# tmaklin/ntcomp

Hardware: AMD Instinct MI355X
Metric: encode Mbases/sec at k=91, 150bp reads, 1/2/4/8 MI355X; bit-exact vs CPU (higher is better)
Workload: dtype u32; 1 GPU; C91: 10000000 x 150bp synthetic reads per GPU (1% subst, 50% revcomp) vs SBWT of a 5 Mbp synthetic genome (+revcomp), k=91; k=91, read_len=150, genome_bp=5000000, err_ppm=10000, reads_per_gpu=10000000, batch_reads=10000000, index_nodes=10000001, records_per_gpu=39278538, suffix_table_u=14, spill_reruns=0, parallelism=reads sharded over 1 GPU(s), index replicated, no collective, inflight=2

## Files before the change

### ntcomp_amd/csrc/capi.cpp

```cpp
#include <hip/hip_runtime.h>

#include <algorithm>
#include <chrono>
#include <cstdio>
#include <cstdlib>
#include <cstring>
#include <exception>
#include <memory>
#include <string>
#include <vector>

#include "../../include/ntcomp_gpu.h"
#include "../../include/ntcomp_codec.h"
#include "../../include/ntcomp_host.h"
#include "codec_params.h"
#include "derived.h"
#include "kernels.h"
#include "nonacgt_core.h"
#include "qrans_core.h"
#include "quality_core.h"
#include "names_core.h"
#include "digest_core.h"
#include "pair_core.h"
#include "window_core.h"
// ... 132 lines not shown
    Enc4Args last4{};
    struct {
        const uint8_t *bases;
        const uint64_t *offs;
        uint64_t n_reads, total_bases, cap;
        uint64_t *rec_out, *rec_offs;
    } call4{};
    uint32_t ent_slots_opt = 0;
    double epool_per_read = 4.0;
    double rpool_per_read = 1.0;
    double epool_per_base = 0.0;
    double rpool_per_base = 0.0;
    uint64_t spill_reruns = 0;
    uint32_t tab_u_opt = 0;
    int tab_u_fallback = 0;
    int pair_bytes_opt = 1;
    int filter_opt = -1;
    int64_t filter_density_ppm = -1;
    int joint_opt = -1;
    int path_link_opt = path_link_on() ? 1 : 0;
    int win_opt = -1;
    int subst_opt = subst_on() ? -1 : 0;
    int subst_built = 0;
    int decode_only_opt = 0;
    bool index_decode_only = false;
    int ext2_opt = 0;
    uint64_t n_paths = 0, path_text_len = 0;
    int64_t upload_host_us = 0, upload_total_us = 0;
    uint64_t max_pass_bases = 1ULL << 30;
    double last_pack_ms = 0;
    NxState nx;
    QualState qual;
    NameState names;
    DigestState dig;
    PairState pair;
    WindowState win;
    int discard_text = 0;
    FastqArgs fq_last{};
    hipEvent_t pack_ev[3] = {nullptr, nullptr, nullptr};
};

namespace {

constexpr uint64_t kCounterBytes = 8 * 64 + 2 * 64;

#define HIP_TRY(ctx, expr)                                                                   \
// ... 1092 lines not shown

int ntc_index_upload(ntc_ctx *ctx, const ntc_index_view *v) {
    if (!ctx || !view_ok(v)) return set_err(ctx, NTC_ERR_INVALID_ARG, "null index view");
    ntc_index_prep p;
    std::string err;
    const int rc = prepare_index(v, p, err);
    if (rc) return set_err(ctx, rc, err);
    return upload_prepared(ctx, p);
}

}

namespace {
struct Upload {
    ntc_ctx *ctx;
    const HostIndex &hx;
    const Derived &dv;
    const uint64_t n;
    const int64_t host_us;
    const std::chrono::steady_clock::time_point t_start = std::chrono::steady_clock::now();
    void *d_lines = nullptr, *d_lcs = nullptr, *d_uniq = nullptr, *d_walk = nullptr;
    void *d_walk_a = nullptr, *d_walk_b = nullptr, *d_pred = nullptr, *d_code = nullptr;
    void *d_pstream = nullptr, *d_colex_at = nullptr, *d_pos = nullptr, *d_puniq = nullptr;
    bool has_paths = false;
    uint64_t tlen = 0, n_paths = 0;
    uint32_t U = 0;
    void *d_tab = nullptr, *d_bits = nullptr, *d_fbits = nullptr;

    Upload(ntc_ctx *c, const ntc_index_prep &p) : ctx(c), hx(p.hx), dv(p.dv), n(p.hx.n), host_us(p.host_us) {}
    int dalloc(uint64_t bytes, void **p) {
        HIP_TRY(ctx, hipMalloc(p, bytes));
        ctx->index_mem->ptrs.push_back(*p);
        ctx->index_bytes += bytes;
        return NTC_OK;
    }
    double seconds() const { return std::chrono::duration<double>(std::chrono::steady_clock::now() - t_start).count(); }
    void mark(const char *what, bool sync) const {
        static const bool trace = std::getenv("NTC_UPLOAD_TRACE") != nullptr;
        if (!trace) return;
        if (sync) (void)hipStreamSynchronize(ctx->stream);
        std::fprintf(stderr, "[upload] %-28s %.4f s\n", what, seconds());
    }
};

int up_free_previous(Upload &u) {
    ntc_ctx *ctx = u.ctx;
    HIP_TRY(ctx, hipStreamSynchronize(ctx->stream));
// ... 98 lines not shown
        uint32_t np32 = 0;
        HIP_TRY(ctx, hipMemcpyAsync(&u.tlen, (uint64_t *)d_base + n, 8, hipMemcpyDeviceToHost, ctx->stream));
        HIP_TRY(ctx, hipMemcpyAsync(&np32, cnt + 1, 4, hipMemcpyDeviceToHost, ctx->stream));
        HIP_TRY(ctx, hipStreamSynchronize(ctx->stream));
        HIP_TRY(ctx, hipGetLastError());
        u.n_paths = np32;
        const uint64_t tlen = u.tlen;
        if (tlen + 64 < (1ULL << 31)) {
            const uint64_t n_groups = (tlen + hx.k) / 32 + 8, n_colex = tlen + 8, n_puniq = tlen / 64 + 4;
            if ((rc = u.dalloc(n_puniq * 8, &u.d_puniq)) || (rc = u.dalloc(n_groups * 16, &u.d_pstream)) ||
                (rc = u.dalloc(n_colex * 4 + 64, &u.d_colex_at)) || (rc = u.dalloc(n * 4, &u.d_pos))) {
                free_tmp();
                return rc;
            }
            HIP_TRY(ctx, hipMemsetAsync(u.d_puniq, 0, n_puniq * 8, ctx->stream));
            HIP_TRY(ctx, hipMemsetAsync(u.d_pstream, 0, n_groups * 16, ctx->stream));
            HIP_TRY(ctx, hipMemsetAsync(u.d_colex_at, 0xFF, n_colex * 4 + 64, ctx->stream));
            HIP_TRY(ctx, hipMemsetAsync(u.d_pos, 0xFF, n * 4, ctx->stream));
            launch_path_place(pa, st, prv, (const uint64_t *)d_base, (uint32_t *)u.d_colex_at, (uint32_t *)u.d_pos,
                              (uint4 *)u.d_pstream, (uint64_t *)u.d_puniq, ctx->stream);
            if (hx.k >= kForkBlockMinK)
                launch_path_forks(pa, st, (const uint32_t *)d_len, (const uint64_t *)d_base, (const uint32_t *)u.d_pos,
                                  (const uint4 *)u.d_pstream, (uint32_t *)u.d_colex_at, ctx->stream);
            HIP_TRY(ctx, hipGetLastError());
            u.has_paths = true;
        }
        free_tmp();
    }
    u.mark("path cover", true);
    HIP_TRY(ctx, hipStreamSynchronize(ctx->stream));
    HIP_TRY(ctx, hipFree(u.d_walk_a));
    HIP_TRY(ctx, hipFree(u.d_walk_b));
    HIP_TRY(ctx, hipFree(u.d_pred));
    HIP_TRY(ctx, hipFree(u.d_code));
    return NTC_OK;
}

int up_joint_choice(Upload &u) {
    ntc_ctx *ctx = u.ctx;
    const bool has_paths = u.has_paths;
    DevIndex &d = ctx->dix;
    d = DevIndex{};
    d.rank = (const uint2 *)u.d_lines;
    d.lcs = (const uint8_t *)u.d_lcs;
    d.uniq = (const uint32_t *)u.d_uniq;
    d.walk = (const WalkEntry *)u.d_walk;
    d.rwords = u.dv.rwords;
    d.n = (uint32_t)u.n;
    d.k = u.hx.k;
    d.t_jump = u.dv.t_jump;
    for (int c = 0; c < 5; c++) d.C[c] = u.dv.C[c];
    d.has_paths = has_paths ? 1u : 0u;
    d.path_len = has_paths ? (uint32_t)u.tlen : 0u;
    d.pstream = (const uint4 *)u.d_pstream;
    d.colex_at = (const uint32_t *)u.d_colex_at;
    d.pos_of_node = (const uint32_t *)u.d_pos;
    d.puniq = (const uint64_t *)u.d_puniq;
    d.forks = has_paths && u.hx.k >= kForkBlockMinK ? 1u : 0u;
    d.absent = u.dv.absent;
    d.joint = has_paths && (ctx->joint_opt == 1 || (ctx->joint_opt < 0 && u.n_paths * kJointAutoNodesPerPath > u.n))
                  ? 1u : 0u;
    return NTC_OK;
}

int up_suffix_table(Upload &u) {
    ntc_ctx *ctx = u.ctx;
    DevIndex &d = ctx->dix;
    const uint64_t n = u.n;
    int rc;
    if (ctx->ext2_opt) {
        void *d_r2;
        if ((rc = u.dalloc(rank2_blocks(n) * 4 * sizeof(Rank2Chunk), &d_r2))) return rc;
        launch_rank2(d, (Rank2Chunk *)d_r2, ctx->stream);
        d.rank2 = (const Rank2Chunk *)d_r2;
    }
    uint32_t U = ctx->tab_u_opt ? std::min<uint32_t>(ctx->tab_u_opt, std::min<uint32_t>(u.hx.k, kTabMaxU))
                                : default_tab_u(n, u.hx.k, u.hx.lcs.data());
    ctx->tab_u_fallback = 0;
    if (!ctx->tab_u_opt && U > 14) {
        size_t free_b = 0, total_b = 0;
        if (hipMemGetInfo(&free_b, &total_b) == hipSuccess &&
// ... 172 lines not shown
    uint64_t t = 0;
    for (const auto &b : ctx->ws) t += b.bytes;
    *value = (int64_t)t;
    return NTC_OK;
}

#define OPT_SET(member) [](ntc_ctx *c, int64_t v) { c->member = (decltype(c->member))v; return (int)NTC_OK; }
#define OPT_GET(expr) [](const ntc_ctx *c, int64_t *v) { *v = (int64_t)(expr); return (int)NTC_OK; }
#define OPT_VALUE(member) OPT_SET(member), OPT_GET(c->member)
#define OPT_UPLOAD(member, built) OPT_SET(member), OPT_GET(c->has_index ? (int64_t)(built) : (int64_t)c->member)
#define OPT_READ(key, expr) {key, 0, 0, kInRange, nullptr, nullptr, OPT_GET(expr)}
#define OPT_DEV(f) {"dev_" #f, 0, 0, kInRange, nullptr, nullptr, \
                    [](const ntc_ctx *c, int64_t *v) { return get_dev_addr(c, c->dix.f, v); }}

const Option kOptions[] = {
    {"encode_variant", 1, 4, kEndsOnly, "encode_variant must be 4 (default) or 1 (A/B baseline)", OPT_VALUE(encode_variant)},
    {"tab_u", 0, kTabMaxU, kInRange, "tab_u must be 0 (default) or 1..15", OPT_UPLOAD(tab_u_opt, c->dix.tab_u)},
    {"pair_bytes", 0, 1, kInRange, "pair_bytes must be 0 or 1", OPT_UPLOAD(pair_bytes_opt, c->dix.pair_w != nullptr)},
    {"filter", -1, 1, kInRange, "filter must be -1 (auto), 0 or 1", OPT_UPLOAD(filter_opt, c->dix.filt_f != 0)},
    {"joint", -1, 1, kInRange, "joint must be -1 (auto), 0 or 1", OPT_UPLOAD(joint_opt, c->dix.joint)},
    {"path_link", 0, 1, kInRange, "path_link must be 0 or 1", OPT_VALUE(path_link_opt)},
    {"win", -1, 1, kInRange, "win must be -1 (auto), 0 or 1", OPT_UPLOAD(win_opt, c->dix.win_w != nullptr)},
    {"subst", -1, 0, kInRange, "subst must be -1 (auto) or 0", OPT_UPLOAD(subst_opt, c->subst_built)},
    {"decode_only", 0, 1, kInRange, "decode_only must be 0 or 1", OPT_UPLOAD(decode_only_opt, c->index_decode_only)},
    {"ext2", 0, 1, kInRange, "ext2 must be 0 or 1", OPT_UPLOAD(ext2_opt, c->dix.rank2 != nullptr)},
    {"warm_dma", 1, 1ll << 30, kInRange, "warm_dma: 1 .. 2^30 bytes", warm_dma, nullptr},
    {"max_pass_bases", 1, kNoMax, kInRange, "max_pass_bases must be >= 1", OPT_VALUE(max_pass_bases)},
    {"ent_slots", 0, 1024, kMultipleOf4, "ent_slots must be 0 (auto) or a multiple of 4 up to 1024", OPT_SET(ent_slots_opt),
     OPT_GET(ent_slots(c))},
    {"pool_per_read", 0, kNoMax, kInRange, "pool_per_read must be >= 0", set_pool_per_read, nullptr},
    {"qualities", 0, 2, kInRange, "qualities must be 0 (drop), 1 (keep) or 2 (bin8)", OPT_VALUE(qual.mode)},
    {"quality_coder", 0, 1, kInRange, "quality_coder must be 0 (pack) or 1 (rans)", OPT_VALUE(qual.coder)},
    {"names", 0, 2, kInRange, "names must be 0 (drop), 1 (keep) or 2 (id)", OPT_VALUE(names.mode)},
    {"discard_text", 0, 1, kInRange, "discard_text must be 0 or 1", OPT_VALUE(discard_text)},
    {"paired", 0, 2, kInRange, "paired must be 0 (off), 1 (ids) or 2 (no check)", OPT_VALUE(pair.mode)},
    {"digests", 0, 1, kInRange, "digests must be 0 or 1", OPT_VALUE(dig.opt)},
    {"non_acgt", 0, 2, kInRange, "non_acgt must be 0 (error), 1 (mask) or 2 (keep)", OPT_VALUE(nx.policy)},
    {"subst_hash", 0, 0, kInRange, nullptr, nullptr, get_subst_hash},
    {"path_hash", 0, 0, kInRange, nullptr, nullptr, get_path_hash},
    {"workspace_bytes", 0, 0, kInRange, nullptr, nullptr, get_workspace_bytes},
    OPT_DEV(walk), OPT_DEV(rank2), OPT_DEV(tab), OPT_DEV(tab_bits),
    OPT_DEV(filt_bits),
    OPT_DEV(pair_w), OPT_DEV(win_w),
    OPT_READ("filter_density_ppm", c->filter_density_ppm),
    OPT_READ("n_paths", c->n_paths),
    OPT_READ("path_text_len", c->path_text_len),
// ... 1517 lines not shown
```

### ntcomp_amd/csrc/derived.cpp

```cpp
#include "derived.h"

#include <algorithm>
#include <cmath>
#include <cstdlib>
#include <string>
#include <thread>

namespace ntc {

bool build_derived(const HostIndex &ix, Derived &out, std::string &err, bool host_paths) {
    const uint64_t n = ix.n;
    const uint32_t k = ix.k;
    if (n == 0 || n >= (uint64_t)kTabShort) {
        err = "index must have 1 <= n < 2^32 - 256 nodes";
        return false;
    }
    if (k < 1 || k > 255) {
        err = "k must be in [1, 255]";
        return false;
    }
    const uint64_t nw = (n + 63) / 64;
    for (int c = 0; c < 4; c++)
        if (ix.rows[c].size() < nw) {
            err = "subset-matrix row shorter than ceil(n/64) words";
// ... 174 lines not shown
    if (!head || !alone || m == 0 || (m & (m - 1))) return kNoNode;
    const int c = __builtin_ctz(m);
    const uint32_t y = dv.C[c] + host_rank(dv, c, z);
    return dummy[y] ? kNoNode : y;
}

void fork_words(const HostIndex &ix, const Derived &dv, const std::vector<uint8_t> &dummy, uint32_t v, uint32_t *w) {
    uint64_t h = v;
    while (h > 0 && ix.lcs[h] >= ix.k - 1) h--;
    const uint32_t m = labels_of(dv, h);
    for (int c = 0; c < 4; c++) {
        w[c] = kNoNode;
        if (!((m >> c) & 1u)) continue;
        const uint32_t y = dv.C[c] + host_rank(dv, c, h);
        if (!dummy[y]) w[c] = dv.pos_of_node[y];
    }
}

bool subst_on() {
    const char *e = std::getenv("NTC_SUBST");
    return !(e && std::atoi(e) == 0);
}

bool path_link_on() {
    const char *e = std::getenv("NTC_PATH_LINK");
    return !(e && std::atoi(e) == 0);
}

void link_unitigs(const HostIndex &ix, const Derived &dv, const std::vector<uint8_t> &dummy,
                  std::vector<uint32_t> &nxt, std::vector<uint32_t> &prv) {
    const uint64_t n = ix.n;
    const uint32_t k = ix.k;
    std::vector<uint32_t> ulen(n, 0);
    for (uint64_t z = 1; z < n; z++) {
        if (dummy[z] || prv[z] != kNoNode) continue;
        uint32_t c = 0;
        for (uint32_t y = (uint32_t)z; y != kNoNode; y = nxt[y]) c++;
        for (uint32_t y = (uint32_t)z; y != kNoNode; y = nxt[y]) ulen[y] = c;
    }
    std::vector<uint64_t> best_pred(n, UINT64_MAX);
    std::vector<uint32_t> want(n, kNoNode);
    for (uint64_t t = 1; t < n; t++) {
        if (dummy[t] || !ulen[t] || nxt[t] != kNoNode) continue;
        uint64_t h = t;
        while (h > 0 && ix.lcs[h] >= k - 1) h--;
        const uint32_t m = labels_of(dv, h);
        uint64_t best = UINT64_MAX;
        const uint64_t mine = (uint64_t)ulen[t] << 32 | t;
        for (int c = 0; c < 4; c++) {
            if (!((m >> c) & 1u)) continue;
            const uint32_t y = dv.C[c] + host_rank(dv, c, h);
            if (dummy[y] || prv[y] != kNoNode || !ulen[y]) continue;
            best = std::min(best, (uint64_t)ulen[y] << 32 | y);
            best_pred[y] = std::min(best_pred[y], mine);
        }
        if (best != UINT64_MAX) want[t] = (uint32_t)best;
    }
    for (uint64_t t = 1; t < n; t++) {
        const uint32_t y = want[t];
        if (y != kNoNode && best_pred[y] == ((uint64_t)ulen[t] << 32 | t)) {
            nxt[t] = y;
            prv[y] = (uint32_t)t;
        }
    }
}

void build_paths(const HostIndex &ix, Derived &dv) {
    const uint64_t n = ix.n;
    const uint32_t k = ix.k;
    dv.has_paths = false;
    if (n >= (1ULL << 31) || k < 1) return;
    const std::vector<uint8_t> dummy = dummy_nodes(ix, dv);
    std::vector<uint32_t> nxt(n), prv(n, kNoNode);
    for (uint64_t z = 0; z < n; z++) {
        nxt[z] = path_succ(ix, dv, dummy, z);
        if (nxt[z] != kNoNode) prv[nxt[z]] = (uint32_t)z;
    }
    if (path_link_on()) link_unitigs(ix, dv, dummy, nxt, prv);
    std::vector<uint8_t> start(n, 0), seen(n, 0);
    for (uint64_t z = 1; z < n; z++)
        if (!dummy[z] && prv[z] == kNoNode) {
            start[z] = 1;
            for (uint32_t y = (uint32_t)z; y != kNoNode; y = nxt[y]) seen[y] = 1;
        }
    for (uint64_t z = 1; z < n; z++)
        if (!dummy[z] && !seen[z]) {
            start[z] = 1;
            for (uint32_t y = (uint32_t)z; !seen[y]; y = nxt[y]) seen[y] = 1;
        }
    std::vector<uint64_t> path_start;
    std::vector<uint32_t> order;
    order.reserve(n);
    for (uint64_t z = 1; z < n; z++) {
// ... 20 lines not shown
    uint64_t b = 0;
    std::vector<uint8_t> first(k);
    for (uint64_t p = 0; p < np; p++) {
        const uint64_t a = path_start[p], e = path_start[p + 1];
        uint32_t z = order[a];
        for (int64_t t = (int64_t)k - 1; t >= 0; t--) {
            first[t] = dv.code[z];
            z = dv.pred[z];
        }
        for (uint32_t t = 0; t < k; t++) put(b + t, first[t]);
        for (uint64_t i = a; i < e; i++) {
            const uint32_t node = order[i];
            const uint64_t pos = b + (i - a);
            if (i > a) put(pos + k - 1, dv.code[node]);
            const uint32_t u = (dv.uniq[node >> 5] >> (node & 31)) & 1u;
            dv.colex_at[pos] = node | (u << 31);
            dv.pos_of_node[node] = (uint32_t)pos;
            const uint64_t end = pos + k - 1;
            dv.pstream[end >> 5].z |= 1u << (end & 31);
            if (u) dv.puniq[pos >> 6] |= 1ULL << (pos & 63);
        }
        b += (e - a) + k;
    }
    if (k >= kForkBlockMinK) {
        b = 0;
        for (uint64_t p = 0; p < np; p++) {
            const uint64_t a = path_start[p], e = path_start[p + 1];
            const uint64_t pos = b + (e - a) - 1;
            uint32_t w[4];
            fork_words(ix, dv, dummy, order[e - 1], w);
            uint32_t *blk = dv.colex_at.data() + fork_block(pos + 1);
            for (int c = 0; c < 4; c++) {
                uint64_t chars = 0;
                uint32_t ends = 0;
                if (w[c] != kNoNode) path_text32(dv.pstream.data(), (uint64_t)w[c] + k - 1, chars, ends);
                blk[4 * c] = w[c];
                blk[4 * c + 1] = (uint32_t)chars;
                blk[4 * c + 2] = (uint32_t)(chars >> 32);
                blk[4 * c + 3] = ends;
            }
            b += (e - a) + k;
        }
    }
    dv.tlen = tlen;
    dv.n_paths = np;
    dv.has_paths = true;
// ... 32 lines not shown
    const uint64_t lines = rank2_blocks(d.n);
    out.resize(lines * 4);
    for (uint64_t i = 0; i < lines * 4; i++) out[i] = rank2_make(d, i % lines, (int)(i / lines));
}

DevIndex host_dev_index(const HostIndex &ix, const Derived &dv, const std::vector<WalkEntry> &walk) {
    DevIndex d{};
    d.rank = dv.rank.data();
    d.lcs = ix.lcs.data();
    d.uniq = dv.uniq.data();
    d.walk = walk.data();
    d.rwords = dv.rwords;
    d.n = (uint32_t)ix.n;
    d.k = ix.k;
    d.t_jump = dv.t_jump;
    for (int c = 0; c < 5; c++) d.C[c] = dv.C[c];
    d.has_paths = dv.has_paths ? 1u : 0u;
    d.path_len = dv.has_paths ? (uint32_t)(dv.colex_at.size() - 8) : 0u;
    d.pstream = dv.pstream.empty() ? nullptr : dv.pstream.data();
    d.colex_at = dv.colex_at.empty() ? nullptr : dv.colex_at.data();
    d.pos_of_node = dv.pos_of_node.empty() ? nullptr : dv.pos_of_node.data();
    d.puniq = dv.puniq.empty() ? nullptr : dv.puniq.data();
    d.forks = dv.has_paths && ix.k >= kForkBlockMinK ? 1u : 0u;
    d.absent = dv.absent;
    d.tab = nullptr;
    d.tab_u = 0;
    return d;
}

}
```

### ntcomp_amd/csrc/derived.h

```cpp
#pragma once
#include <cstdint>
#include <vector>

#include "encode_core.h"
#include "ntc_internal.h"

namespace ntc {

struct Derived {
    uint32_t rwords = 0;
    std::vector<uint2> rank;
    std::vector<uint32_t> uniq;
    std::vector<uint32_t> pred;
    std::vector<uint8_t> code;
    uint32_t C[5] = {0, 0, 0, 0, 0};
    uint32_t t_jump = 1;
    bool has_paths = false;
    uint64_t tlen = 0;
    std::vector<uint4> pstream;
    std::vector<uint32_t> colex_at;
    std::vector<uint32_t> pos_of_node;
    std::vector<uint64_t> puniq;
    uint64_t n_paths = 0;
    uint32_t absent = 0;
};

constexpr uint32_t kNoNode = 0xFFFFFFFFu;

void build_paths(const HostIndex &ix, Derived &dv);
bool path_link_on();
bool subst_on();
inline uint64_t path_cover_hash(const uint4 *pstream, const uint32_t *colex_at, const uint32_t *pos_of_node,
                                const uint64_t *puniq, uint64_t n, uint32_t k, uint64_t tlen) {
    uint64_t h = 1469598103934665603ULL;
    auto mix = [&](const void *p, uint64_t bytes) {
        const uint8_t *b = (const uint8_t *)p;
        for (uint64_t i = 0; i < bytes; i++) h = (h ^ b[i]) * 1099511628211ULL;
    };
    for (uint64_t g = 0; g < pstream_groups(tlen, k); g++) mix(pstream + g, 12);
    mix(colex_at, (tlen + 8) * 4);
    mix(pos_of_node, n * 4);
    mix(puniq, (tlen / 64 + 4) * 8);
    return h;
}
inline uint64_t subst_word_hash(const uint4 *pstream, uint64_t groups) {
    uint64_t h = 1469598103934665603ULL;
    for (uint64_t g = 0; g < groups; g++)
        for (uint32_t i = 0; i < 4; i++) h = (h ^ ((pstream[g].w >> (8 * i)) & 0xFFu)) * 1099511628211ULL;
    return h;
}
std::vector<uint8_t> dummy_nodes(const HostIndex &ix, const Derived &dv);
uint32_t default_tab_u(uint64_t n, uint32_t k, const uint8_t *lcs = nullptr);
// ... 11 lines not shown
```

### ntcomp_amd/csrc/encode_core.h

```cpp
#pragma once
#include <hip/hip_runtime.h>

#include <cstdint>

#define NTC_HD __host__ __device__ __forceinline__
typedef uint32_t u32x4_t __attribute__((ext_vector_type(4)));
#ifndef NTC_NT
#define NTC_NT 17
#endif

#if defined(NTC_TRACE) && !defined(__HIP_DEVICE_COMPILE__)
void ntc_touch(int kind, const void *p);
#define NTC_TOUCH(kind, p) ntc_touch(kind, (const void *)(p))
#else
#define NTC_TOUCH(kind, p) ((void)0)
#endif
enum { kTrRank, kTrLcs, kTrUniq, kTrTabU, kTrTabLo, kTrBits, kTrFilt, kTrColex, kTrPon, kTrPst, kTrQ, kTrE,
       kTrPuniq, kTrEw, kTrKinds };

namespace ntc {

#if defined(NTC_STATS) && !defined(__HIP_DEVICE_COMPILE__)
extern uint64_t ntc_stats[16];
#define NTC_STAT(i) (ntc_stats[i]++)
// ... 17 lines not shown
    uint32_t jump;
    uint32_t older;
};
NTC_HD WalkEntry walk_compose(const WalkStep &x, const WalkStep &y, const WalkStep &z) {
    WalkEntry e;
    e.w0 = x.chars;
    e.w1 = (y.chars >> 32) | ((uint64_t)x.older << 32);
    e.w2 = (uint64_t)y.older | ((y.chars & 0xFFFFFFFFull) << 32);
    e.older = (uint32_t)z.chars;
    e.jump = z.jump;
    return e;
}

struct alignas(64) Rank2Chunk {
    uint32_t base;
    uint32_t bits;
    uint32_t pbase[4];
    uint32_t pbits[4];
    uint32_t pad[6];
};
static_assert(sizeof(Rank2Chunk) == 64, "rank2 chunk");
NTC_HD uint64_t rank2_blocks(uint64_t n) { return (n >> 5) + 2; }

struct DevIndex {
    const uint2 *rank;
    const uint8_t *lcs;
    const uint32_t *uniq;
    const WalkEntry *walk;
    uint32_t rwords;
    uint32_t n;
    uint32_t k;
    uint32_t t_jump;
    uint32_t C[5];
    uint32_t has_paths;
    const uint4 *pstream;
    const uint32_t *colex_at;
    const uint32_t *pos_of_node;
    const uint64_t *puniq;
    const uint2 *tab;
    const uint32_t *tab_bits;
    const uint32_t *filt_bits;
    uint32_t filt_f;
    const uint16_t *pair_w;
    uint32_t path_len;
    uint32_t tab_pos;
    uint32_t tab_u;
    uint32_t absent;
    const Rank2Chunk *rank2;
    uint32_t joint;
    const uint32_t *win_w;
    uint32_t forks;
};

constexpr uint32_t kForkBlockMinK = 19;
NTC_HD uint64_t fork_block(uint64_t t) { return (t + 3) & ~3ull; }
NTC_HD void path_text32(const uint4 *pstream, uint64_t T, uint64_t &chars, uint32_t &ends) {
    const uint4 g0 = pstream[T >> 5], g1 = pstream[(T >> 5) + 1];
    const uint32_t sh = (uint32_t)(T & 31);
    const uint64_t c0 = (uint64_t)g0.x | ((uint64_t)g0.y << 32), c1 = (uint64_t)g1.x | ((uint64_t)g1.y << 32);
    chars = sh ? ((c0 >> (2 * sh)) | (c1 << (64 - 2 * sh))) : c0;
    ends = sh ? ((g0.z >> sh) | (g1.z << (32 - sh))) : g0.z;
}

enum : int {
    kErrInvalidBase = 2,
    kErrEmptyRead = 3,
    kErrLength = 4,
    kErrCapacity = 5,
    kErrFormat = 8,
    kErrRefPanic = 11,
};

NTC_HD int base_code(uint8_t b) {
    switch (b) {
    case 'A': return 0;
// ... 530 lines not shown
    load_w2(w + i, a, b);
    return sh ? ((a >> sh) | (b << (64 - sh))) : a;
}
NTC_HD uint64_t window1(const uint64_t *w, uint32_t off) {
    const uint32_t i = off >> 6, sh = off & 63;
    const uint64_t a = w[i];
    return sh ? ((a >> sh) | (w[i + 1] << (64 - sh))) : a;
}
NTC_HD uint32_t ctz64(uint64_t x) { return x ? (uint32_t)__builtin_ctzll(x) : 64u; }
NTC_HD uint32_t uniq_bit(const DevIndex &ix, uint32_t v) {
    NTC_TOUCH(kTrUniq, ix.uniq + (v >> 5));
    return (ix.uniq[v >> 5] >> (v & 31)) & 1u;
}

NTC_HD void tab_ds(const DevIndex &ix, const uint64_t *Q, uint64_t qo, uint32_t x, uint32_t &d, uint32_t &s) {
    const uint32_t u = x + 1 < ix.tab_u ? x + 1 : ix.tab_u;
    const uint64_t key = window2(Q, qo + x + 1 - u) & ((1ULL << (2 * u)) - 1);
    NTC_TOUCH(u == ix.tab_u ? kTrTabU : kTrTabLo, ix.tab + tab_base(u) + key);
    const uint2 e = ix.tab[tab_base(u) + key];
    d = tab_long(e) ? u : (e.y & 0xFFu);
    s = e.x;
}

#ifndef NTC_ONES_PAIR
#define NTC_ONES_PAIR 0
#endif
NTC_HD uint32_t ones_down(const uint64_t *w, uint32_t a, uint32_t maxn) {
    uint32_t cnt = 0;
    int64_t pos = a;
#if NTC_ONES_PAIR
    {
        const uint32_t wi = (uint32_t)(pos >> 6), b = (uint32_t)(pos & 63);
        NTC_TOUCH(kTrPuniq, w + wi);
        const uint64_t hiw = w[wi], low = w[wi > 0 ? wi - 1 : 0];
        const uint64_t x = ~hiw << (63 - b);
        const uint32_t z = x ? (uint32_t)__builtin_clzll(x) : 64u;
        if (z <= b || wi == 0 || maxn <= b + 1) return (z <= b ? z : b + 1) < maxn ? (z <= b ? z : b + 1) : maxn;
        NTC_TOUCH(kTrPuniq, w + wi - 1);
        cnt = b + 1;
        const uint64_t y = ~low;
        const uint32_t z2 = y ? (uint32_t)__builtin_clzll(y) : 64u;
        if (z2 < 64) { cnt += z2; return cnt < maxn ? cnt : maxn; }
        cnt += 64;
        pos -= b + 1 + 64;
        if (pos < 0) return cnt < maxn ? cnt : maxn;
    }
#endif
    while (cnt < maxn) {
        const uint32_t wi = (uint32_t)(pos >> 6), b = (uint32_t)(pos & 63);
        NTC_TOUCH(kTrPuniq, w + wi);
        const uint64_t x = ~w[wi] << (63 - b);
        const uint32_t z = x ? (uint32_t)__builtin_clzll(x) : 64u;
        if (z <= b) { cnt += z; break; }
        cnt += b + 1;
        pos -= b + 1;
        if (pos < 0) break;
    }
    return cnt < maxn ? cnt : maxn;
}

NTC_HD Entry load_entry(const Entry *E, int32_t i) {
    NTC_TOUCH(kTrE, E + i);
#ifdef __HIP_DEVICE_COMPILE__
    const uint4 v = *reinterpret_cast<const uint4 *>(E + i);
    return Entry{v.x, v.y, v.z, v.w};
#else
    return E[i];
#endif
}

// ... 65 lines not shown
        if (!have) eg = at(g);
#else
        Entry eg = at(g);
        while (g + 1 < e) {
            const Entry nx = at(g + 1);
            if (nx.p > x) break;
            g++;
            eg = nx;
        }
#endif
        e = g;
        cur = eg;
    }
    NTC_HD bool covered(uint32_t x) {
        seek(x);
        return e >= 0 && cur.p <= x && x < cur.p + cur.m;
    }
    NTC_HD uint32_t dval(const Entry &en, uint32_t x) const {
        const uint32_t d0 = en.dk & 0xFFu;
        const uint32_t d = d0 + (x - en.p);
        return (en.dk & kRunTag) ? (d < k ? d : k) : d0;
    }
    NTC_HD uint32_t sval(const Entry &en, uint32_t x) const {
        if (en.dk & kRunTag) NTC_TOUCH(kTrColex, ix->colex_at + en.v + (x - en.p));
        return (en.dk & kRunTag) ? (ix->colex_at[en.v + (x - en.p)] & 0x7FFFFFFFu) : en.v;
    }
    NTC_HD uint32_t D(uint32_t x) {
        if (covered(x)) return dval(cur, x);
        uint32_t d, s;
        tab_ds(*ix, Q, qo, x, d, s);
        return d;
    }
    NTC_HD void DS(uint32_t x, uint32_t &d, uint32_t &s) {
        if (covered(x)) {
            d = dval(cur, x);
            s = (d > 11 || d == k) ? sval(cur, x) : 0u;
        } else {
            tab_ds(*ix, Q, qo, x, d, s);
        }
    }
    NTC_HD uint32_t run_from(uint32_t x, uint32_t cap) const {
        int32_t c = e;
        uint32_t cnt = 0;
        int64_t pos = x;
        Entry en = cur;
        while (cnt < cap && pos >= 0) {
            while (c > 0 && en.p > (uint32_t)pos) en = at(--c);
            if (!(c >= 0 && en.p <= (uint32_t)pos && (uint32_t)pos < en.p + en.m)) {
                if (ix->tab_u != k || (uint32_t)pos + 1 < k) break;
                uint32_t d, s;
                tab_ds(*ix, Q, qo, (uint32_t)pos, d, s);
                if (d != k || !uniq_bit(*ix, s)) break;
                cnt++;
                pos--;
                continue;
            }
            const uint32_t d0 = en.dk & 0xFFu;
            if (!(en.dk & kRunTag)) {
                if (d0 != k || !uniq_bit(*ix, en.v)) break;
                cnt++;
                pos--;
                continue;
            }
            const uint32_t tx = (uint32_t)pos - en.p;
            const uint32_t tk = d0 >= k ? 0u : k - d0;
            if (tx < tk) break;
            const uint32_t want = tx - tk + 1;
            const uint32_t got = ones_down(ix->puniq, en.v + tx, want);
// ... 447 lines not shown
                            put_entry(b, p, j + 1, m, (d + 1 < k ? d + 1 : k) | kRunTag);
                            p += m;
                            d = d + m < k ? d + m : k;
                            j += m;
                            if (jy() != 0xFFFFFFFFu) jy() += m;
                            vfy = (4u + c + (lx > lim ? 0u : 8u) + (ly > lim ? 0u : 16u)) << 8;
                            try_run = true;
                            return 0;
                        }
                    }
                    break;
                }
            }
            if (kJoint && jy() != 0xFFFFFFFFu) {
                if (m > 0) {
                    put_entry(b, p, j + 1, m, (d + 1 < k ? d + 1 : k) | kRunTag);
                    p += m;
                    d = d + m < k ? d + m : k;
                    if (p >= len) { jy() = 0xFFFFFFFFu; return 1; }
                }
                if (m > 0 || nohop) {
                    NTC_TOUCH(kTrColex, ix.colex_at + j + m);
                    NTC_TOUCH(kTrColex, ix.colex_at + jy() + m);
                    l = ld_hint<256>(ix.colex_at + j + m) & 0x7FFFFFFFu;
                    r = (ld_hint<256>(ix.colex_at + jy() + m) & 0x7FFFFFFFu) + 1;
#if defined(NTC_STATS) && !defined(__HIP_DEVICE_COMPILE__)
                    if (p < len) {
                        const int c = (int)((Q[(qo + p) >> 5] >> (2 * ((qo + p) & 31))) & 3u);
                        const bool el = (ix.rank[(uint64_t)c * ix.rwords + (l >> 5)].y >> (l & 31)) & 1u;
                        const bool er = (ix.rank[(uint64_t)c * ix.rwords + ((r - 1) >> 5)].y >> ((r - 1) & 31)) & 1u;
                        NTC_STAT(el && er ? 8 : (el || er ? 9 : 10));
                    }
#endif
                }
                jy() = 0xFFFFFFFFu;
                m = 0;
                nohop = false;
            }
            if (!kJoint && unc && m == 0) {
                NTC_STAT(14);
                j = gj;
                p = ge;
                d = (unc >> 1) & 0xFFu;
                window(b, p + 1 - U);
                mode = kModeBrk;
            }
            if (m > 0 || nohop) {
                if (m > 0) {
                    put_entry(b, p, j + 1, m, (d + 1 < k ? d + 1 : k) | kRunTag);
                    p += m;
                    j += m;
                    d = d + m < k ? d + m : k;
                    if (p >= len) return 1;
                }
                gj = j;
                ge = p;
#if defined(NTC_STATS) && !defined(__HIP_DEVICE_COMPILE__)
                {
                    const uint32_t v = ix.colex_at[j] & 0x7FFFFFFFu;
                    const int c = (int)((Q[(qo + p) >> 5] >> (2 * ((qo + p) & 31))) & 3u);
                    NTC_STAT(((ix.rank[(uint64_t)c * ix.rwords + (v >> 5)].y >> (v & 31)) & 1u) ? 11 : 12);
                }
#endif
                if constexpr (!kJoint) {
                    if (sub && d + 1 >= U && p + U + 1 < len) {
                        NTC_STAT(13);
                        vfy = U | (1u << 8) | (d << 9);
                        j = gj + U + 1;
                        jy() = 0xFFFFFFFFu;
                        p = ge + U + 1;
                        d = U;
                        hi = kScanW;
                        try_run = true;
                        mode = kModeBrk;
                        return 0;
                    }
                }
                window(b, p + 1 - U);
                mode = kModeBrk;
#if !NTC_CHAIN
                return 0;
#endif
// ... 299 lines not shown
                tested = cand;
            }
            uint32_t longm = 0;
#pragma unroll
            for (uint32_t i = 0; i < kScanW; i++)
                if ((tested >> i) & 1u) {
                    const uint64_t key = key_at(p + i, U);
                    NTC_TOUCH(kTrBits, ix.tab_bits + (key >> 5));
                    longm |= ((ld_hint<2>(ix.tab_bits + (key >> 5)) >> (key & 31)) & 1u) << i;
                }
            const uint32_t pairs = longm & (longm >> 1);
            if (pairs == 0) {
                if (p + span >= len) { p = len; return 1; }
                p += span - ((longm >> (span - 1)) & 1u);
                return 0;
            }
            const uint32_t x = p + (uint32_t)__builtin_ctz(pairs);
            NTC_TOUCH(kTrTabU, ix.tab + tab_base(U) + key_at(x, U));
            return enter_pair(ix, b, x, load2_stream(ix.tab + tab_base(U) + key_at(x, U)));
        }
        if (!covers(p + 1 - U, p)) window(b, p + 1 - U);
        if (mode == kModeBrkLong) {
            NTC_TOUCH(kTrColex, ix.colex_at + j);
            l = ld_hint<256>(ix.colex_at + j) & 0x7FFFFFFFu;
            r = l + 1;
            mode = kModeExt;
#if !NTC_CHAIN
            return 0;
#endif
        }
        if (mode == kModeEnter) {
            if (!covers(p - U, p - 1)) window(b, p - U);
            NTC_TOUCH(kTrTabU, ix.tab + tab_base(U) + key_at(p - 1, U));
            return enter_pair(ix, b, p - 1, load2_stream(ix.tab + tab_base(U) + key_at(p - 1, U)));
        }
        if (mode == kModeBrk) {
#if NTC_BRK_PAIR
            if (ix.pair_w) {
                const uint64_t M = key_at(p - 1, U - 1);
                const uint32_t c = (uint32_t)(qw >> (2 * (p - qb))) & 3u;
                NTC_TOUCH(kTrBits, ix.pair_w + M);
                NTC_TOUCH(kTrColex, ix.colex_at + j);
                const uint32_t pw = ld_hint<32>(ix.pair_w + M);
                const uint32_t v = ld_hint<256>(ix.colex_at + j) & 0x7FFFFFFFu;
                if (!((pw >> (4 + c)) & 1u)) {
                    p += 1;
                    mode = kModeScan;
                    hi = U + 1 < kScanW ? U + 1 : kScanW;
                    return p >= len ? 1 : 0;
                }
                l = v;
                r = v + 1;
                mode = kModeExt;
                return 0;
            }
#endif
            NTC_TOUCH(kTrTabU, ix.tab + tab_base(U) + key_at(p, U));
            const uint2 te = load2_stream(ix.tab + tab_base(U) + key_at(p, U));
            NTC_TOUCH(kTrColex, ix.colex_at + j);
            const uint32_t v = ld_hint<256>(ix.colex_at + j) & 0x7FFFFFFFu;
            if (!tab_long(te)) {
                skip_short(b, te, U);
                return p >= len ? 1 : 0;
            }
            l = v;
            r = v + 1;
            mode = kModeExt;
            return 0;
        }
        const int c = (int)((qw >> (2 * (p - qb))) & 3u);
        if (mode == kModeExt && ix.rank2 && p + 1 < len && p + 1 < qb + 32) {
            const int c2 = (int)((qw >> (2 * (p + 1 - qb))) & 3u);
            uint32_t l1, r1, l2, r2;
            extend2(ix, c, c2, l, r, l1, r1, l2, r2);
            if (l1 < r1) {
                const uint32_t d1 = d + 1 < k ? d + 1 : k;
                put_entry(b, p, l1, 1u, d1);
                p++;
                if (l2 < r2) return commit(ix, b, l2, r2, d1 + 1 < k ? d1 + 1 : k);
                l = l1; r = r1; d = d1;
                mode = kModeExtFail;
                return 0;
            }
// ... 74 lines not shown
    uint64_t *pool;
    uint64_t cap;
    unsigned long long *cnt;
    uint32_t *rbase;
    unsigned long long *status;
    uint64_t rid;
};

NTC_HD int parse_read(const DevIndex &ix, const uint64_t *Q, uint64_t qo, const Entry *E, uint32_t ne,
                      uint32_t len, uint64_t *slot, uint64_t *spill, uint64_t sstride = 1,
                      const Entry *Ed = nullptr, uint64_t es = 1, const Entry *pre = nullptr,
                      const Entry *E2 = nullptr, uint32_t S = kNoLimit, const RecPool *rp = nullptr) {
    const uint32_t k = ix.k;
    EntryView ev(E, &ix, Q, qo, k, (int32_t)ne - 1, Ed, es, pre, E2, S);
    uint32_t i = len;
    int nrec = 0;
    while (i > 0) {
        const uint32_t x = i - 1;
        uint32_t di, st;
        ev.DS(x, di, st);
        const uint32_t segend = i;
        uint32_t seglen;
        if (di == k && i > k + 1) {
            const uint32_t ext = ev.run_from(i - 2, i - k - 1);
            const uint32_t L = k + ext;
            uint32_t m = L, pp = i;
            for (;;) {
                const uint32_t dp = ev.D(pp - 1);
                if (dp < m) {
                    if (dp >= pp || dp == 0) return -kErrFormat;
                    m -= dp;
                    pp -= dp;
                } else {
                    break;
                }
            }
            seglen = L - (m - 1);
            i = pp;
        } else {
            if (di == 0) return -kErrFormat;
            seglen = di;
            if (i > di) i -= di - 1;
            else i = 0;
        }
        if (seglen >= (1u << 24)) return -kErrLength;
        const uint64_t first = nrec == 0 ? 1u : 0u;
        uint64_t w;
        if (seglen > 11) {
            w = (uint64_t)st | ((uint64_t)(seglen & 0xFFFFFFu) << 32) | (first << 56);
        } else {
            if (seglen > k) return -kErrRefPanic;
            NTC_TOUCH(kTrQ, Q + ((qo + segend - seglen) >> 5));
            const uint64_t bits = window2(Q, qo + segend - seglen);
            w = (bits & ((1ULL << (2 * seglen)) - 1)) | ((uint64_t)((first + 2) | (seglen << 2)) << 56);
        }
        if (nrec < (int)kRecSlot) {
            slot[(uint64_t)nrec * sstride] = w;
        } else {
            if (rp && nrec == (int)kRecSlot) {
                const uint64_t need = 1 + (uint64_t)i;
#ifdef __HIP_DEVICE_COMPILE__
                const uint64_t at = atomicAdd(rp->cnt, (unsigned long long)need);
#else
                const uint64_t at = *rp->cnt;
                *rp->cnt += need;
#endif
                if (at + need <= rp->cap) {
                    rp->rbase[rp->rid] = (uint32_t)at;
                    spill = rp->pool + at - kRecSlot;
                } else {
                    spill = nullptr;
#ifdef __HIP_DEVICE_COMPILE__
// ... 158 lines not shown
```

### ntcomp_amd/csrc/kernels.h

```cpp
#pragma once
#include <hip/hip_runtime.h>

#include <cstdint>
#include <string>
#include <vector>

#include "encode_core.h"

namespace ntc {

struct HostIndex;
struct BuildOpts {
    uint64_t device_budget = 0, host_budget = 0, max_partition_keys = 0;
    std::string temp_dir;
};
struct BuildStats {
    uint64_t occurrences = 0, kmers = 0, sources = 0, nodes = 0;
    uint64_t spilled_bytes = 0, device_budget = 0, pass_keys = 0, peak_device_bytes = 0;
    uint32_t kmer_partitions = 0, node_partitions = 0, compactions = 0, seq_uploads = 0;
    double seconds = 0, seconds_kmers = 0, seconds_sources = 0, seconds_nodes = 0, seconds_labels = 0;
    double seconds_plan = 0, seconds_sort = 0;
};
bool build_index_device(hipStream_t s, const uint8_t *seqs, const uint64_t *offs, uint64_t n_seqs, uint32_t k,
                        bool revcomp, const BuildOpts &o, HostIndex &out, BuildStats &st, std::string &err);
// ... 398 lines not shown
};
void launch_status_box(const unsigned long long *status, const uint64_t *a, const uint64_t *b, const uint64_t *c,
                       uint64_t *box, hipStream_t s);
void launch_walk_build(const uint32_t *pred, const uint8_t *code, uint64_t n, WalkStep *a, WalkStep *b,
                       WalkEntry *out, hipStream_t s);
uint64_t scan_tmp_words(uint64_t n);

struct PathArgs {
    const uint2 *rank;
    uint32_t rwords;
    uint32_t n, k;
    const uint8_t *lcs;
    const uint32_t *dummy;
    const uint32_t *pred;
    const uint8_t *code;
    const uint32_t *uniq;
};
void launch_path_edges(const PathArgs &a, uint32_t *prv, hipStream_t s);
uint4 *launch_path_rank(const uint32_t *prv, uint32_t n, uint4 *a, uint4 *b, hipStream_t s);
void launch_path_link(const PathArgs &a, const uint4 *st, const uint32_t *len, uint32_t *want,
                      unsigned long long *best_pred, uint32_t *prv, hipStream_t s);
void launch_path_forks(const PathArgs &a, const uint4 *st, const uint32_t *len, const uint64_t *base,
                       const uint32_t *pos_of_node, const uint4 *pstream, uint32_t *colex_at, hipStream_t s);
void launch_path_cut(const PathArgs &a, const uint4 *st, uint32_t *prv, uint32_t *flag, hipStream_t s);
void launch_path_lengths(const PathArgs &a, const uint4 *st, const uint32_t *prv, uint32_t *len, uint32_t *vals,
                         uint32_t *n_paths, hipStream_t s);
void launch_path_place(const PathArgs &a, const uint4 *st, const uint32_t *prv, const uint64_t *base,
                       uint32_t *colex_at, uint32_t *pos_of_node, uint4 *pstream, uint64_t *puniq, hipStream_t s);
void scan_excl_u32(const uint32_t *in, uint64_t n, uint64_t *out, uint64_t *tmp, hipStream_t s);
void scan_excl_u64(const uint64_t *in, uint64_t n, uint64_t *out, uint64_t *tmp, hipStream_t s);

}
```

### ntcomp_amd/csrc/kernels.hip

```cpp
#include <hip/hip_runtime.h>

#include <cstdint>

#include "encode_core.h"
#include "kernels.h"

namespace ntc {

__global__ __launch_bounds__(256) void k_encode(EncodeArgs a) {
    const uint64_t gid = (uint64_t)blockIdx.x * 256 + threadIdx.x;
    if (gid >= a.n_reads) return;
    const uint64_t tile = gid >> 6;
    const uint32_t lane = (uint32_t)(gid & 63);
    uint64_t base, rows;
    if (a.tile_base) {
        base = a.tile_base[tile];
        rows = a.tile_base[tile + 1] - base;
    } else {
        base = tile * a.rows_uniform;
        rows = a.rows_uniform;
    }
    const uint64_t beg = a.offs[gid], end = a.offs[gid + 1];
    const uint64_t len64 = end >= beg ? end - beg : 0;
    LaneScratch s;
// ... 1099 lines not shown
    uint32_t h = z;
    while (h > 0 && a.lcs[h] >= a.k - 1) h--;
    uint4 *blk = reinterpret_cast<uint4 *>(colex_at + fork_block(pos + 1));
#pragma unroll
    for (int c = 0; c < 4; c++) {
        const uint2 w = a.rank[(uint64_t)c * a.rwords + (h >> 5)];
        uint32_t v = 0xFFFFFFFFu;
        if ((w.y >> (h & 31)) & 1u) {
            const uint32_t y = rank_word(w, h);
            if (!path_dummy(a.dummy, y)) v = pos_of_node[y];
        }
        uint64_t chars = 0;
        uint32_t ends = 0;
        if (v != 0xFFFFFFFFu) path_text32(pstream, (uint64_t)v + a.k - 1, chars, ends);
        blk[c] = make_uint4(v, (uint32_t)chars, (uint32_t)(chars >> 32), ends);
    }
}

void launch_path_forks(const PathArgs &a, const uint4 *st, const uint32_t *len, const uint64_t *base,
                       const uint32_t *pos_of_node, const uint4 *pstream, uint32_t *colex_at, hipStream_t s) {
    hipLaunchKernelGGL(k_path_forks, grid_for(a.n), dim3(256), 0, s, a, st, len, base, pos_of_node, pstream, colex_at);
}

void launch_path_edges(const PathArgs &a, uint32_t *prv, hipStream_t s) {
    hipLaunchKernelGGL(k_path_edges, grid_for(a.n), dim3(256), 0, s, a, prv);
}

uint4 *launch_path_rank(const uint32_t *prv, uint32_t n, uint4 *a, uint4 *b, hipStream_t s) {
    hipLaunchKernelGGL(k_path_rank_init, grid_for(n), dim3(256), 0, s, prv, n, a);
    int rounds = 1;
    while ((1ull << rounds) < (uint64_t)n) rounds++;
    for (int r = 0; r < rounds; r++) {
        hipLaunchKernelGGL(k_path_rank_step, grid_for(n), dim3(256), 0, s, (const uint4 *)a, n, b);
        std::swap(a, b);
    }
    return a;
}

void launch_path_cut(const PathArgs &a, const uint4 *st, uint32_t *prv, uint32_t *flag, hipStream_t s) {
    hipLaunchKernelGGL(k_path_cut, grid_for(a.n), dim3(256), 0, s, a, st, prv, flag);
}

void launch_path_lengths(const PathArgs &a, const uint4 *st, const uint32_t *prv, uint32_t *len, uint32_t *vals,
                         uint32_t *n_paths, hipStream_t s) {
    hipLaunchKernelGGL(k_path_len, grid_for(a.n), dim3(256), 0, s, a, st, len);
    hipLaunchKernelGGL(k_path_vals, grid_for(a.n), dim3(256), 0, s, a, prv, (const uint32_t *)len, vals, n_paths);
// ... 10 lines not shown
```

Baseline: 383,900 Mbases/s.

## Pack unique-run length hints into colex_at high bits to shortcut run_from

Adds an index-build step, on both device and host, that stores a 2-bit code for the preceding unique-run length (32/64/128) in bits 29-30 of colex_at entries. During encode, run_from uses this floor to return or skip ahead without walking the puniq bitmap word by word. All node loads now mask with a per-index node_mask so the extra bits are stripped. This adds an index-build kernel and lowers the node-id limit to 2^29. It also removes the dead NTC_ONES_PAIR path and adds a stat counter in the hot loop.

After: 394,200 Mbases/s, median of 6. 1.03x the previous value.

```diff
diff --git a/ntcomp_amd/csrc/capi.cpp b/ntcomp_amd/csrc/capi.cpp
--- a/ntcomp_amd/csrc/capi.cpp
+++ b/ntcomp_amd/csrc/capi.cpp
@@ -178,6 +178,7 @@
     int win_opt = -1;
     int subst_opt = subst_on() ? -1 : 0;
     int subst_built = 0;
+    int uniq_hint_opt = uniq_hint_on() ? -1 : 0;
     int decode_only_opt = 0;
     bool index_decode_only = false;
     int ext2_opt = 0;
@@ -1316,7 +1317,7 @@
     void *d_lines = nullptr, *d_lcs = nullptr, *d_uniq = nullptr, *d_walk = nullptr;
     void *d_walk_a = nullptr, *d_walk_b = nullptr, *d_pred = nullptr, *d_code = nullptr;
     void *d_pstream = nullptr, *d_colex_at = nullptr, *d_pos = nullptr, *d_puniq = nullptr;
-    bool has_paths = false;
+    bool has_paths = false, uniq_hint = false;
     uint64_t tlen = 0, n_paths = 0;
     uint32_t U = 0;
     void *d_tab = nullptr, *d_bits = nullptr, *d_fbits = nullptr;
@@ -1461,6 +1462,11 @@
             if (hx.k >= kForkBlockMinK)
                 launch_path_forks(pa, st, (const uint32_t *)d_len, (const uint64_t *)d_base, (const uint32_t *)u.d_pos,
                                   (const uint4 *)u.d_pstream, (uint32_t *)u.d_colex_at, ctx->stream);
+            if (ctx->uniq_hint_opt != 0 && n <= kUniqHintMaxN) {
+                launch_path_hint(hx.k, tlen, (const uint4 *)u.d_pstream, (const uint64_t *)u.d_puniq,
+                                 (uint32_t *)u.d_colex_at, ctx->stream);
+                u.uniq_hint = true;
+            }
             HIP_TRY(ctx, hipGetLastError());
             u.has_paths = true;
         }
@@ -1496,6 +1502,8 @@
     d.pos_of_node = (const uint32_t *)u.d_pos;
     d.puniq = (const uint64_t *)u.d_puniq;
     d.forks = has_paths && u.hx.k >= kForkBlockMinK ? 1u : 0u;
+    d.uniq_hint = has_paths && u.uniq_hint ? 1u : 0u;
+    d.node_mask = d.uniq_hint ? kNodeMaskHint : kNodeMaskPlain;
     d.absent = u.dv.absent;
     d.joint = has_paths && (ctx->joint_opt == 1 || (ctx->joint_opt < 0 && u.n_paths * kJointAutoNodesPerPath > u.n))
                   ? 1u : 0u;
@@ -1714,6 +1722,7 @@
     {"path_link", 0, 1, kInRange, "path_link must be 0 or 1", OPT_VALUE(path_link_opt)},
     {"win", -1, 1, kInRange, "win must be -1 (auto), 0 or 1", OPT_UPLOAD(win_opt, c->dix.win_w != nullptr)},
     {"subst", -1, 0, kInRange, "subst must be -1 (auto) or 0", OPT_UPLOAD(subst_opt, c->subst_built)},
+    {"uniq_hint", -1, 0, kInRange, "uniq_hint must be -1 (auto) or 0", OPT_UPLOAD(uniq_hint_opt, c->dix.uniq_hint)},
     {"decode_only", 0, 1, kInRange, "decode_only must be 0 or 1", OPT_UPLOAD(decode_only_opt, c->index_decode_only)},
     {"ext2", 0, 1, kInRange, "ext2 must be 0 or 1", OPT_UPLOAD(ext2_opt, c->dix.rank2 != nullptr)},
     {"warm_dma", 1, 1ll << 30, kInRange, "warm_dma: 1 .. 2^30 bytes", warm_dma, nullptr},
diff --git a/ntcomp_amd/csrc/derived.cpp b/ntcomp_amd/csrc/derived.cpp
--- a/ntcomp_amd/csrc/derived.cpp
+++ b/ntcomp_amd/csrc/derived.cpp
@@ -220,6 +220,11 @@
     return !(e && std::atoi(e) == 0);
 }
 
+bool uniq_hint_on() {
+    const char *e = std::getenv("NTC_UNIQ_HINT");
+    return !(e && std::atoi(e) == 0);
+}
+
 bool path_link_on() {
     const char *e = std::getenv("NTC_PATH_LINK");
     return !(e && std::atoi(e) == 0);
@@ -263,10 +268,11 @@
     }
 }
 
-void build_paths(const HostIndex &ix, Derived &dv) {
+void build_paths(const HostIndex &ix, Derived &dv, bool hint, uint64_t hint_max_n) {
     const uint64_t n = ix.n;
     const uint32_t k = ix.k;
     dv.has_paths = false;
+    dv.uniq_hint = false;
     if (n >= (1ULL << 31) || k < 1) return;
     const std::vector<uint8_t> dummy = dummy_nodes(ix, dv);
     std::vector<uint32_t> nxt(n), prv(n, kNoNode);
@@ -333,6 +339,14 @@
         }
         b += (e - a) + k;
     }
+    if (hint && n <= hint_max_n) {
+        uint32_t r = 0;
+        for (uint64_t j = 0; j < tlen; j++) {
+            if (dv.colex_at[j] != kNoNode) dv.colex_at[j] |= uniq_code(r) << kUniqShift;
+            r = ((dv.puniq[j >> 6] >> (j & 63)) & 1u) ? (r < 128 ? r + 1 : r) : 0u;
+        }
+        dv.uniq_hint = true;
+    }
     if (k >= kForkBlockMinK) {
         b = 0;
         for (uint64_t p = 0; p < np; p++) {
@@ -411,6 +425,8 @@
     d.pos_of_node = dv.pos_of_node.empty() ? nullptr : dv.pos_of_node.data();
     d.puniq = dv.puniq.empty() ? nullptr : dv.puniq.data();
     d.forks = dv.has_paths && ix.k >= kForkBlockMinK ? 1u : 0u;
+    d.uniq_hint = dv.has_paths && dv.uniq_hint ? 1u : 0u;
+    d.node_mask = d.uniq_hint ? kNodeMaskHint : kNodeMaskPlain;
     d.absent = dv.absent;
     d.tab = nullptr;
     d.tab_u = 0;
diff --git a/ntcomp_amd/csrc/derived.h b/ntcomp_amd/csrc/derived.h
--- a/ntcomp_amd/csrc/derived.h
+++ b/ntcomp_amd/csrc/derived.h
@@ -22,12 +22,15 @@
     std::vector<uint32_t> pos_of_node;
     std::vector<uint64_t> puniq;
     uint64_t n_paths = 0;
+    bool uniq_hint = false;
     uint32_t absent = 0;
 };
 
 constexpr uint32_t kNoNode = 0xFFFFFFFFu;
 
-void build_paths(const HostIndex &ix, Derived &dv);
+bool uniq_hint_on();
+void build_paths(const HostIndex &ix, Derived &dv, bool hint = uniq_hint_on(),
+                 uint64_t hint_max_n = kUniqHintMaxN);
 bool path_link_on();
 bool subst_on();
 inline uint64_t path_cover_hash(const uint4 *pstream, const uint32_t *colex_at, const uint32_t *pos_of_node,
diff --git a/ntcomp_amd/csrc/encode_core.h b/ntcomp_amd/csrc/encode_core.h
--- a/ntcomp_amd/csrc/encode_core.h
+++ b/ntcomp_amd/csrc/encode_core.h
@@ -63,6 +63,7 @@
 static_assert(sizeof(Rank2Chunk) == 64, "rank2 chunk");
 NTC_HD uint64_t rank2_blocks(uint64_t n) { return (n >> 5) + 2; }
 
+constexpr uint32_t kNodeMaskPlain = 0x7FFFFFFFu, kNodeMaskHint = 0x1FFFFFFFu;
 struct DevIndex {
     const uint2 *rank;
     const uint8_t *lcs;
@@ -91,7 +92,14 @@
     uint32_t joint;
     const uint32_t *win_w;
     uint32_t forks;
+    uint32_t node_mask = kNodeMaskPlain;
+    uint32_t uniq_hint = 0;
 };
+
+constexpr uint64_t kUniqHintMaxN = 1ull << 29;
+constexpr uint32_t kUniqShift = 29;
+NTC_HD uint32_t uniq_code(uint32_t r) { return r >= 128 ? 3u : (r >= 64 ? 2u : (r >= 32 ? 1u : 0u)); }
+NTC_HD uint32_t uniq_floor(uint32_t code) { return (0x80402000u >> (8 * code)) & 0xFFu; }
 
 constexpr uint32_t kForkBlockMinK = 19;
 NTC_HD uint64_t fork_block(uint64_t t) { return (t + 3) & ~3ull; }
@@ -668,30 +676,9 @@
     s = e.x;
 }
 
-#ifndef NTC_ONES_PAIR
-#define NTC_ONES_PAIR 0
-#endif
 NTC_HD uint32_t ones_down(const uint64_t *w, uint32_t a, uint32_t maxn) {
     uint32_t cnt = 0;
     int64_t pos = a;
-#if NTC_ONES_PAIR
-    {
-        const uint32_t wi = (uint32_t)(pos >> 6), b = (uint32_t)(pos & 63);
-        NTC_TOUCH(kTrPuniq, w + wi);
-        const uint64_t hiw = w[wi], low = w[wi > 0 ? wi - 1 : 0];
-        const uint64_t x = ~hiw << (63 - b);
-        const uint32_t z = x ? (uint32_t)__builtin_clzll(x) : 64u;
-        if (z <= b || wi == 0 || maxn <= b + 1) return (z <= b ? z : b + 1) < maxn ? (z <= b ? z : b + 1) : maxn;
-        NTC_TOUCH(kTrPuniq, w + wi - 1);
-        cnt = b + 1;
-        const uint64_t y = ~low;
-        const uint32_t z2 = y ? (uint32_t)__builtin_clzll(y) : 64u;
-        if (z2 < 64) { cnt += z2; return cnt < maxn ? cnt : maxn; }
-        cnt += 64;
-        pos -= b + 1 + 64;
-        if (pos < 0) return cnt < maxn ? cnt : maxn;
-    }
-#endif
     while (cnt < maxn) {
         const uint32_t wi = (uint32_t)(pos >> 6), b = (uint32_t)(pos & 63);
         NTC_TOUCH(kTrPuniq, w + wi);
@@ -803,8 +790,12 @@
         return (en.dk & kRunTag) ? (d < k ? d : k) : d0;
     }
     NTC_HD uint32_t sval(const Entry &en, uint32_t x) const {
+        const uint32_t s = sval_coded(en, x);
+        return (en.dk & kRunTag) ? (s & ix->node_mask) : s;
+    }
+    NTC_HD uint32_t sval_coded(const Entry &en, uint32_t x) const {
         if (en.dk & kRunTag) NTC_TOUCH(kTrColex, ix->colex_at + en.v + (x - en.p));
-        return (en.dk & kRunTag) ? (ix->colex_at[en.v + (x - en.p)] & 0x7FFFFFFFu) : en.v;
+        return (en.dk & kRunTag) ? (ix->colex_at[en.v + (x - en.p)] & kNodeMaskPlain) : en.v;
     }
     NTC_HD uint32_t D(uint32_t x) {
         if (covered(x)) return dval(cur, x);
@@ -815,16 +806,30 @@
     NTC_HD void DS(uint32_t x, uint32_t &d, uint32_t &s) {
         if (covered(x)) {
             d = dval(cur, x);
-            s = (d > 11 || d == k) ? sval(cur, x) : 0u;
+            s = (d > 11 || d == k) ? sval_coded(cur, x) : 0u;
         } else {
             tab_ds(*ix, Q, qo, x, d, s);
         }
     }
-    NTC_HD uint32_t run_from(uint32_t x, uint32_t cap) const {
+    NTC_HD uint32_t run_from(uint32_t x, uint32_t cap, uint32_t sx = 0) const {
         int32_t c = e;
         uint32_t cnt = 0;
         int64_t pos = x;
         Entry en = cur;
+        const uint32_t T = ix->uniq_hint ? uniq_floor((sx >> kUniqShift) & 3u) : 0u;
+        if (T && e >= 0 && (cur.dk & kRunTag) && cur.p <= x && x < cur.p + cur.m && cap > 0) {
+            const uint32_t d0 = cur.dk & 0xFFu, tx = x - cur.p;
+            const uint32_t tk = d0 >= k ? 0u : k - d0;
+            if (tx < tk) return 0;
+            const uint32_t want = tx - tk + 1;
+            if (T >= want) {
+                if (tk > 0 || want >= cap) return want < cap ? want : cap;
+                cnt = want;
+                pos = (int64_t)cur.p - 1;
+            } else if (T >= cap) {
+                return cap;
+            }
+        }
         while (cnt < cap && pos >= 0) {
             while (c > 0 && en.p > (uint32_t)pos) en = at(--c);
             if (!(c >= 0 && en.p <= (uint32_t)pos && (uint32_t)pos < en.p + en.m)) {
@@ -1318,8 +1323,8 @@
                 if (m > 0 || nohop) {
                     NTC_TOUCH(kTrColex, ix.colex_at + j + m);
                     NTC_TOUCH(kTrColex, ix.colex_at + jy() + m);
-                    l = ld_hint<256>(ix.colex_at + j + m) & 0x7FFFFFFFu;
-                    r = (ld_hint<256>(ix.colex_at + jy() + m) & 0x7FFFFFFFu) + 1;
+                    l = ld_hint<256>(ix.colex_at + j + m) & ix.node_mask;
+                    r = (ld_hint<256>(ix.colex_at + jy() + m) & ix.node_mask) + 1;
 #if defined(NTC_STATS) && !defined(__HIP_DEVICE_COMPILE__)
                     if (p < len) {
                         const int c = (int)((Q[(qo + p) >> 5] >> (2 * ((qo + p) & 31))) & 3u);
@@ -1353,7 +1358,7 @@
                 ge = p;
 #if defined(NTC_STATS) && !defined(__HIP_DEVICE_COMPILE__)
                 {
-                    const uint32_t v = ix.colex_at[j] & 0x7FFFFFFFu;
+                    const uint32_t v = ix.colex_at[j] & ix.node_mask;
                     const int c = (int)((Q[(qo + p) >> 5] >> (2 * ((qo + p) & 31))) & 3u);
                     NTC_STAT(((ix.rank[(uint64_t)c * ix.rwords + (v >> 5)].y >> (v & 31)) & 1u) ? 11 : 12);
                 }
@@ -1699,7 +1704,7 @@
         if (!covers(p + 1 - U, p)) window(b, p + 1 - U);
         if (mode == kModeBrkLong) {
             NTC_TOUCH(kTrColex, ix.colex_at + j);
-            l = ld_hint<256>(ix.colex_at + j) & 0x7FFFFFFFu;
+            l = ld_hint<256>(ix.colex_at + j) & ix.node_mask;
             r = l + 1;
             mode = kModeExt;
 #if !NTC_CHAIN
@@ -1719,7 +1724,7 @@
                 NTC_TOUCH(kTrBits, ix.pair_w + M);
                 NTC_TOUCH(kTrColex, ix.colex_at + j);
                 const uint32_t pw = ld_hint<32>(ix.pair_w + M);
-                const uint32_t v = ld_hint<256>(ix.colex_at + j) & 0x7FFFFFFFu;
+                const uint32_t v = ld_hint<256>(ix.colex_at + j) & ix.node_mask;
                 if (!((pw >> (4 + c)) & 1u)) {
                     p += 1;
                     mode = kModeScan;
@@ -1735,7 +1740,7 @@
             NTC_TOUCH(kTrTabU, ix.tab + tab_base(U) + key_at(p, U));
             const uint2 te = load2_stream(ix.tab + tab_base(U) + key_at(p, U));
             NTC_TOUCH(kTrColex, ix.colex_at + j);
-            const uint32_t v = ld_hint<256>(ix.colex_at + j) & 0x7FFFFFFFu;
+            const uint32_t v = ld_hint<256>(ix.colex_at + j) & ix.node_mask;
             if (!tab_long(te)) {
                 skip_short(b, te, U);
                 return p >= len ? 1 : 0;
@@ -1856,7 +1861,8 @@
         const uint32_t segend = i;
         uint32_t seglen;
         if (di == k && i > k + 1) {
-            const uint32_t ext = ev.run_from(i - 2, i - k - 1);
+            const uint32_t ext = ev.run_from(i - 2, i - k - 1, st);
+            ntc_stat_add(15, (uint64_t)(ext + 1) * i);
             const uint32_t L = k + ext;
             uint32_t m = L, pp = i;
             for (;;) {
@@ -1881,7 +1887,8 @@
         const uint64_t first = nrec == 0 ? 1u : 0u;
         uint64_t w;
         if (seglen > 11) {
-            w = (uint64_t)st | ((uint64_t)(seglen & 0xFFFFFFu) << 32) | (first << 56);
+            const uint32_t node = ix.uniq_hint ? st & kNodeMaskHint : st;
+            w = (uint64_t)node | ((uint64_t)(seglen & 0xFFFFFFu) << 32) | (first << 56);
         } else {
             if (seglen > k) return -kErrRefPanic;
             NTC_TOUCH(kTrQ, Q + ((qo + segend - seglen) >> 5));
diff --git a/ntcomp_amd/csrc/kernels.h b/ntcomp_amd/csrc/kernels.h
--- a/ntcomp_amd/csrc/kernels.h
+++ b/ntcomp_amd/csrc/kernels.h
@@ -444,6 +444,8 @@
                       unsigned long long *best_pred, uint32_t *prv, hipStream_t s);
 void launch_path_forks(const PathArgs &a, const uint4 *st, const uint32_t *len, const uint64_t *base,
                        const uint32_t *pos_of_node, const uint4 *pstream, uint32_t *colex_at, hipStream_t s);
+void launch_path_hint(uint32_t k, uint64_t tlen, const uint4 *pstream, const uint64_t *puniq, uint32_t *colex_at,
+                      hipStream_t s);
 void launch_path_cut(const PathArgs &a, const uint4 *st, uint32_t *prv, uint32_t *flag, hipStream_t s);
 void launch_path_lengths(const PathArgs &a, const uint4 *st, const uint32_t *prv, uint32_t *len, uint32_t *vals,
                          uint32_t *n_paths, hipStream_t s);
diff --git a/ntcomp_amd/csrc/kernels.hip b/ntcomp_amd/csrc/kernels.hip
--- a/ntcomp_amd/csrc/kernels.hip
+++ b/ntcomp_amd/csrc/kernels.hip
@@ -1145,6 +1145,21 @@
     hipLaunchKernelGGL(k_path_forks, grid_for(a.n), dim3(256), 0, s, a, st, len, base, pos_of_node, pstream, colex_at);
 }
 
+__global__ __launch_bounds__(256) void k_path_hint(uint32_t k, uint64_t tlen, const uint4 *pstream,
+                                                   const uint64_t *puniq, uint32_t *colex_at) {
+    const uint64_t j = (uint64_t)blockIdx.x * 256u + threadIdx.x;
+    if (j == 0 || j >= tlen) return;
+    const uint64_t end = j + k - 1;
+    if (!((pstream[end >> 5].z >> (end & 31)) & 1u)) return;
+    const uint32_t code = uniq_code(ones_down(puniq, (uint32_t)(j - 1), 128));
+    if (code) colex_at[j] |= code << kUniqShift;
+}
+
+void launch_path_hint(uint32_t k, uint64_t tlen, const uint4 *pstream, const uint64_t *puniq, uint32_t *colex_at,
+                      hipStream_t s) {
+    hipLaunchKernelGGL(k_path_hint, grid_for(tlen), dim3(256), 0, s, k, tlen, pstream, puniq, colex_at);
+}
+
 void launch_path_edges(const PathArgs &a, uint32_t *prv, hipStream_t s) {
     hipLaunchKernelGGL(k_path_edges, grid_for(a.n), dim3(256), 0, s, a, prv);
 }
```
